# CrystalSixone/VLN-MAGIC

Measured on AMD Instinct MI355X. Metric: trajectory-steps/sec (whole node), MAGIC-S R2R pretrain, higher is better.
Workload: dtype bf16

## Files before the change

### vln-magic_amd/csrc/encoder.hip

```cpp
#include "enc_common.hpp"
#include <cstdlib>
#include <cstring>

template <typename Hh> struct EncLayerT {
  const Hh* Wqkv; const float* bqkv;
  const Hh* Wo; const float* bo; const float* g1; const float* be1;
  const Hh* W1; const float* bi;
  const Hh* W2; const float* bo2; const float* g2; const float* be2;
  Hh *qkv, *P, *Pd, *ctx, *a, *z, *g, *out;
  float *rstd_a, *rstd_o;
  unsigned site_attn, site_ao, site_out, pad_;
};
template <typename Hh> struct EncSegT { const Hh* x; const unsigned char* kmask; int nsamp, N, ldp, nlayers; EncLayerT<Hh> L[6]; };
template <typename Hh> struct EncParamsT {
  EncSegT<Hh> seg[2]; int nseg; float p_attn, p_hidden, eps, scale; const unsigned* seed;
  unsigned* sync; int sync_words, pad2_;
};
typedef EncParamsT<bf16> EncParams; typedef EncSegT<bf16> EncSeg; typedef EncLayerT<bf16> EncLayer;
#define F(f) ABI_VIEW(EncLayer, magic_enc_layer, f)
F(Wqkv) F(bqkv) F(Wo) F(bo) F(g1) F(be1) F(W1) F(bi) F(W2) F(bo2) F(g2) F(be2) F(qkv) F(P) F(Pd) F(ctx) F(a) F(z) F(g) F(out) F(rstd_a) F(rstd_o)
F(site_attn) F(site_ao) F(site_out) F(pad_)
#undef F
#define F(f) ABI_VIEW(EncSeg, magic_enc_seg, f)
F(x) F(kmask) F(nsamp) F(N) F(ldp) F(nlayers) F(L)
// ... 1139 lines not shown
    {
      f32x4 acc[NRT][3];
#pragma unroll
      for (int i = 0; i < NRT; ++i)
#pragma unroll
        for (int ct = 0; ct < 3; ++ct) acc[i][ct] = (f32x4){0.f, 0.f, 0.f, 0.f};
#pragma unroll
      for (int ks = 0; ks < 4; ++ks) {
#pragma unroll
        for (int i = 0; i < NRT; ++i) {
          const h16x8<Hh> a = lfrag(sX, XS, i * 16, ks * 32, lane);
#pragma unroll
          for (int ct = 0; ct < 3; ++ct) acc[i][ct] = emma(a, bw[ct][ks], acc[i][ct]);
        }
        KSTEP_FENCE();
      }
#pragma unroll
      for (int ct = 0; ct < 3; ++ct) {
        const int col = (3 * w + ct) * 16 + c16;
#pragma unroll
        for (int i = 0; i < NRT; ++i)
#pragma unroll
          for (int r = 0; r < 4; ++r) sQKV[(i * 16 + 4 * g + r) * QS + col] = from_f<Hh>(acc[i][ct][r] + pb_qkv[ct]);
      }
    }
    h16x8<Hh> wo[4], wq[4];
#pragma unroll
    for (int ks = 0; ks < 4; ++ks) { wo[ks] = gfrag(L.Wo, EH, w * 16, ks * 32, lane); wq[ks] = gfrag(L.Wq, EH, w * 16, ks * 32, lane); }
    __syncthreads();
    copy_out(sQKV, QS, L.qkv + qbase * 3 * EH, 3 * EH, Nq, 3 * EH, tid);
    dd.site = L.site_attn; dd.p = p.p_attn;
    const DropState dsa = drop_init(dd);
    Hh* sPw = sP + w * 16 * PSW;
    for (int u = w; u < ENH * NRT; u += NWAVE)
      attn_unit<NRT>(sQKV, sPw, sA, L.P, L.Pd, u / NRT, u % NRT, Nq, Nq, sg.ldps, qbias, sg.dist, sw, sb, samp, p.scale, dsa, lane);
    __syncthreads();
    copy_out(sA, XS, L.ctx + qbase * EH, EH, Nq, EH, tid);
    {
      f32x4 acc[NRT];
      proj16<NRT>(acc, sA, wo, lane);
      dd.site = L.site_ao; dd.p = p.p_hidden;
      const DropState dsh = drop_init(dd);
      add_norm<NRT, MAXROWS>(acc, pb_o, pg_1, pe_1, sX, red, sA, L.rstd_a, Nq, qbase, p.eps, dsh, w, lane);
    }
    h16x8<Hh> wkv[2][4];
#pragma unroll
    for (int ct = 0; ct < 2; ++ct)
#pragma unroll
      for (int ks = 0; ks < 4; ++ks) wkv[ct][ks] = gfrag(L.Wkv, EH, (2 * w + ct) * 16, ks * 32, lane);
    __syncthreads();
    copy_out(sA, XS, L.a + qbase * EH, EH, Nq, EH, tid);
    {
      f32x4 acc[NRT];
      proj16<NRT>(acc, sA, wq, lane);
#pragma unroll
      for (int i = 0; i < NRT; ++i)
#pragma unroll
        for (int r = 0; r < 4; ++r) sQKV[(i * 16 + 4 * g + r) * QS + colw] = from_f<Hh>(acc[i][r] + pb_q);
    }
    {
      f32x4 acc[NKT][2];
#pragma unroll
      for (int i = 0; i < NKT; ++i)
#pragma unroll
        for (int ct = 0; ct < 2; ++ct) acc[i][ct] = (f32x4){0.f, 0.f, 0.f, 0.f};
      const Hh* cx = sg.cx + kbase * EH;
#pragma unroll
      for (int ks = 0; ks < 4; ++ks) {
#pragma unroll
        for (int i = 0; i < NKT; ++i) {
          const int row = min(i * 16 + c16, Nk - 1);
          const h16x8<Hh> a = *(const h16x8<Hh>*)(cx + (long long)row * EH + ks * 32 + 8 * g);
#pragma unroll
          for (int ct = 0; ct < 2; ++ct) acc[i][ct] = emma(a, wkv[ct][ks], acc[i][ct]);
        }
        KSTEP_FENCE();
      }
#pragma unroll
      for (int ct = 0; ct < 2; ++ct) {
        const int col = EH + (2 * w + ct) * 16 + c16;
#pragma unroll
        for (int i = 0; i < NKT; ++i)
#pragma unroll
          for (int r = 0; r < 4; ++r) {
            const int row = i * 16 + 4 * g + r;
            sQKV[row * QS + col] = (row < Nk) ? from_f<Hh>(acc[i][ct][r] + pb_kv[ct]) : (Hh)0.0f;
          }
      }
    }
    for (int id = tid; id < (KROWS - NKT * 16) * (256 / 8); id += NWAVE * 64) {
      const int r = NKT * 16 + id / 32, c = EH + (id % 32) * 8;
      h16x8<Hh> zv;
#pragma unroll
      for (int e = 0; e < 8; ++e) zv[e] = (Hh)0.0f;
      *(h16x8<Hh>*)(sQKV + r * QS + c) = zv;
    }
    h16x8<Hh> woc[4];
#pragma unroll
    for (int ks = 0; ks < 4; ++ks) woc[ks] = gfrag(L.Woc, EH, w * 16, ks * 32, lane);
    h16x8<Hh> w1[4][4];
#pragma unroll
    for (int ct = 0; ct < 4; ++ct)
#pragma unroll
      for (int ks = 0; ks < 4; ++ks) w1[ct][ks] = gfrag(L.W1, EH, (4 * w + ct) * 16, ks * 32, lane);
    __syncthreads();
    copy_out(sQKV, QS, L.q + qbase * EH, EH, Nq, EH, tid);
    copy_out(sQKV + EH, QS, L.kv + kbase * 2 * EH, 2 * EH, Nk, 2 * EH, tid);
    dd.site = L.site_cattn; dd.p = p.p_attn;
    const DropState dsc = drop_init(dd);
    for (int u = w; u < ENH * NRT; u += NWAVE)
      attn_unit<NKT>(sQKV, sPw, sX, L.Pc, L.Pdc, u / NRT, u % NRT, Nq, Nk, sg.ldpc, cbias, nullptr, 0.f, 0.f, samp, p.scale, dsc, lane);
    __syncthreads();
    copy_out(sX, XS, L.cctx + qbase * EH, EH, Nq, EH, tid);
    {
      f32x4 acc[NRT];
      proj16<NRT>(acc, sX, woc, lane);
      dd.site = L.site_co; dd.p = p.p_hidden;
      const DropState dsh = drop_init(dd);
      add_norm<NRT, MAXROWS>(acc, pb_oc, pg_c, pe_c, sA, red, sX, L.rstd_c, Nq, qbase, p.eps, dsh, w, lane);
    }
    __syncthreads();
    copy_out(sX, XS, L.c + qbase * EH, EH, Nq, EH, tid);
    h16x8<Hh> w2[16];
    {
      f32x4 acc[NRT][4];
#pragma unroll
      for (int i = 0; i < NRT; ++i)
#pragma unroll
        for (int ct = 0; ct < 4; ++ct) acc[i][ct] = (f32x4){0.f, 0.f, 0.f, 0.f};
#pragma unroll
      for (int ks = 0; ks < 4; ++ks) {
#pragma unroll
        for (int i = 0; i < NRT; ++i) {
          const h16x8<Hh> a = lfrag(sX, XS, i * 16, ks * 32, lane);
#pragma unroll
          for (int ct = 0; ct < 4; ++ct) acc[i][ct] = emma(a, w1[ct][ks], acc[i][ct]);
        }
        KSTEP_FENCE();
      }
#pragma unroll
      for (int ks = 0; ks < 16; ++ks) w2[ks] = gfrag(L.W2, EI, w * 16, ks * 32, lane);
#pragma unroll
      for (int ct = 0; ct < 4; ++ct) {
        const int col = (4 * w + ct) * 16 + c16;
#pragma unroll
        for (int i = 0; i < NRT; ++i)
#pragma unroll
          for (int r = 0; r < 4; ++r) {
            acc[i][ct][r] += pb_ffn[ct];
            sG[(i * 16 + 4 * g + r) * GS + col] = from_f<Hh>(acc[i][ct][r]);
          }
      }
      __syncthreads();
      copy_out(sG, GS, L.z + qbase * EI, EI, Nq, EI, tid);
#pragma unroll
      for (int ct = 0; ct < 4; ++ct)
#pragma unroll
        for (int i = 0; i < NRT; ++i)
#pragma unroll
          for (int r = 0; r < 4; ++r) acc[i][ct][r] = gelu_fast(acc[i][ct][r]);
      __syncthreads();
#pragma unroll
      for (int ct = 0; ct < 4; ++ct) {
        const int col = (4 * w + ct) * 16 + c16;
#pragma unroll
        for (int i = 0; i < NRT; ++i)
#pragma unroll
          for (int r = 0; r < 4; ++r) sG[(i * 16 + 4 * g + r) * GS + col] = from_f<Hh>(acc[i][ct][r]);
      }
    }
    __syncthreads();
    copy_out(sG, GS, L.g + qbase * EI, EI, Nq, EI, tid);
    {
      f32x4 acc[NRT];
#pragma unroll
      for (int i = 0; i < NRT; ++i) acc[i] = (f32x4){0.f, 0.f, 0.f, 0.f};
#pragma unroll
      for (int ks = 0; ks < 16; ++ks) {
#pragma unroll
        for (int i = 0; i < NRT; ++i) acc[i] = emma(lfrag(sG, GS, i * 16, ks * 32, lane), w2[ks], acc[i]);
        if ((ks & 1) == 1) KSTEP_FENCE();
      }
      dd.site = L.site_out; dd.p = p.p_hidden;
      const DropState dsh = drop_init(dd);
      add_norm<NRT, MAXROWS>(acc, pb_2, pg_2, pe_2, sX, red, sX, L.rstd_o, Nq, qbase, p.eps, dsh, w, lane);
    }
    __syncthreads();
    copy_out(sX, XS, L.out + qbase * EH, EH, Nq, EH, tid);
  }
}

template <int NKT, typename Hh>
__device__ __forceinline__ void rs_attn(Hh* sQ, const Hh* sK, const Hh* sV, float* sS, Hh* sPd, const float (&kbias)[NKT], const int Nk, const int kmax,
                                        const float* dist, const float sw, const float sb, const int q0, const int nq, const int Nq,
                                        Hh* Pg, Hh* Pdg, const int ldp, const long long samp, const float scale, const DropState& dsa,
                                        const int tid, const int w, const int lane) {
  const int g = lane >> 4, c16 = lane & 15;
  const int NKP = (Nk + 31) / 32 * 32;
  for (int u = w; u < ENH * NKT; u += NWAVE) {
    const int h = u / NKT, j = u % NKT;
    f32x4 sc = (f32x4){0.f, 0.f, 0.f, 0.f};
#pragma unroll
    for (int ks = 0; ks < 2; ++ks) sc = emma(lfrag(sQ, XS, 0, h * EHD + ks * 32, lane), lfrag(sK, XS, j * 16, h * EHD + ks * 32, lane), sc);
    const int key = j * 16 + c16;
    float mb = 0.f;
#pragma unroll
    for (int jj = 0; jj < NKT; ++jj) mb = (jj == j) ? kbias[jj] : mb;
#pragma unroll
    for (int r = 0; r < 4; ++r) {
      float x = sc[r] * scale + mb;
      if (dist && key < Nk) { const int qrow = min(q0 + 4 * g + r, Nq - 1); x += sw * dist[((long long)samp * Nq + qrow) * Nk + key] + sb; }
      sS[(h * 16 + 4 * g + r) * RS_SS + key] = key < Nk ? x : -3.0e38f;
    }
  }
  __syncthreads();
  {
    const int rr = 4 * w + g, h = rr >> 4, ql = rr & 15;
    float e[NKT], mx = -3.0e38f;
#pragma unroll
    for (int j = 0; j < NKT; ++j) { e[j] = sS[rr * RS_SS + j * 16 + c16]; mx = fmaxf(mx, e[j]); }
    mx = g16_max(mx);
    float sum = 0.f;
#pragma unroll
    for (int j = 0; j < NKT; ++j) { e[j] = (j * 16 + c16) < Nk ? __expf(e[j] - mx) : 0.f; sum += e[j]; }
    sum = 1.0f / g16_sum(sum);
    Hh* pc = (Hh*)(sS + rr * RS_SS);
    Hh* pd = sPd + rr * RS_PP;
#pragma unroll
    for (int j = 0; j < NKT; ++j) {
      const int key = j * 16 + c16;
      const float pv = e[j] * sum;
      pc[key] = from_f<Hh>(pv);
      if (dsa.on) {
        const unsigned idx = (unsigned)(((((long long)samp * ENH + h) * Nq + q0 + ql) * Nk) + key);
        pd[key] = from_f<Hh>((ql < nq && key < Nk) ? pv * drop_mul(dsa, idx) : 0.f);
      }
    }
    if (NKT * 16 < NKP && c16 < NKP - NKT * 16) { pc[NKT * 16 + c16] = (Hh)0.0f; if (dsa.on) pd[NKT * 16 + c16] = (Hh)0.0f; }
  }
  __syncthreads();
  {
    const int cpr = ldp / 8;
    for (int id = tid; id < ENH * nq * cpr; id += NWAVE * 64) {
      const int h = id / (nq * cpr), rem = id % (nq * cpr), r = rem / cpr, c = (rem % cpr) * 8;
      const long long go = (((long long)samp * ENH + h) * Nq + q0 + r) * ldp + c;
      *(h16x8<Hh>*)(Pg + go) = *(const h16x8<Hh>*)((const Hh*)(sS + (h * 16 + r) * RS_SS) + c);
      if (dsa.on && Pdg) *(h16x8<Hh>*)(Pdg + go) = *(const h16x8<Hh>*)(sPd + (h * 16 + r) * RS_PP + c);
    }
  }
  {
    const int h = w >> 2, jd = w & 3;
    const Hh* pa = dsa.on ? sPd + h * 16 * RS_PP : (const Hh*)(sS + h * 16 * RS_SS);
    const int pp = dsa.on ? RS_PP : 2 * RS_SS;
    f32x4 o = (f32x4){0.f, 0.f, 0.f, 0.f};
    for (int ks = 0; ks < NKP / 32; ++ks)
      o = emma(lfrag(pa, pp, 0, ks * 32, lane), tfrag_clamp(sV + h * EHD, XS, jd * 16, ks * 32, lane, kmax), o);
#pragma unroll
    for (int r = 0; r < 4; ++r) sQ[(4 * g + r) * XS + h * EHD + jd * 16 + c16] = from_f<Hh>(o[r]);
  }
  __syncthreads();
}

template <int NRT, typename Hh>
__device__ __forceinline__ void xenc_rs_body(const XParamsT<Hh>& p, const XSegT<Hh>& sg, const int samp, const int tile, const int ntile,
                                             unsigned* cnt, unsigned* err, unsigned char* smem) {
  constexpr int NKT = 5;
  Hh* sK = (Hh*)smem;
  Hh* sV = sK + 80 * XS;
  Hh* sU = sV + 81 * XS;
  Hh* sX = sU;
  float* sS = (float*)sU;
  Hh* sPd = sU + 2 * 16 * RS_SS * 2;
  Hh* sG = sU;
  Hh* sZ = sK;
  Hh* sQ = sU + 80 * XS;
  Hh* sO = sQ + 16 * XS;
  Hh* sA = sO + 16 * XS;
  float* red = (float*)(sA + 16 * XS);
  const int tid = threadIdx.x, lane0 = tid & 63, w = __builtin_amdgcn_readfirstlane(tid >> 6);
  const int Nq = sg.Nq, Nk = sg.Nk;
  const long long qbase = (long long)samp * Nq, kbase = (long long)samp * Nk;
  const int r0 = tile * 16, nq = min(16, Nq - r0);
  const long long row0 = qbase + r0;
  if (tid < XS / 8) {
    h16x8<Hh> zv;
#pragma unroll
    for (int e = 0; e < 8; ++e) zv[e] = (Hh)0.0f;
    *(h16x8<Hh>*)(sV + RS_ZROW * XS + tid * 8) = zv;
  }
  DropDesc dd;
  dd.seed = p.seed;
  float qbias[NRT], cbias[NKT];
#pragma unroll
  for (int j = 0; j < NRT; ++j) {
    const int key = j * 16 + (lane0 & 15);
    qbias[j] = (key < Nq && sg.qmask && !sg.qmask[qbase + key]) ? -10000.0f : 0.f;
  }
#pragma unroll
  for (int j = 0; j < NKT; ++j) {
    const int key = j * 16 + (lane0 & 15);
    cbias[j] = (key < Nk && sg.cmask && !sg.cmask[kbase + key]) ? -10000.0f : 0.f;
  }
  const float sw = sg.dist ? sg.sprel_w[0] : 0.f, sb = sg.dist ? sg.sprel_b[0] : 0.f;
  for (int l = 0; l < sg.nlayers; ++l) {
    const XLayerT<Hh>& L = sg.L[l];
    int lane = lane0;
    asm volatile("" : "+v"(lane));
    const int g = lane >> 4, c16 = lane & 15;
    const int colw = w * 16 + c16;
    const float pb_q0 = L.bqkv[colw], pb_kv0 = L.bqkv[EH + (2 * w) * 16 + c16], pb_kv1 = L.bqkv[EH + (2 * w + 1) * 16 + c16];
    const float pb_ck0 = L.bkv[(2 * w) * 16 + c16], pb_ck1 = L.bkv[(2 * w + 1) * 16 + c16];
    float pb_ffn[4];
#pragma unroll
    for (int ct = 0; ct < 4; ++ct) pb_ffn[ct] = L.bi[(4 * w + ct) * 16 + c16];
    const float pb_o = L.bo[colw], pg_1 = L.g1[colw], pe_1 = L.be1[colw], pb_q = L.bq[colw];
    const float pb_oc = L.boc[colw], pg_c = L.gc[colw], pe_c = L.bec[colw];
    const float pb_2 = L.bo2[colw], pg_2 = L.g2[colw], pe_2 = L.be2[colw];
    h16x8<Hh> wq[4], wkv[2][4];
#pragma unroll
    for (int ks = 0; ks < 4; ++ks) {
      wq[ks] = gfrag(L.Wqkv, EH, w * 16, ks * 32, lane);
      wkv[0][ks] = gfrag(L.Wqkv, EH, EH + (2 * w) * 16, ks * 32, lane);
      wkv[1][ks] = gfrag(L.Wqkv, EH, EH + (2 * w + 1) * 16, ks * 32, lane);
    }
    if (l > 0) {
      if (tid == 0) {
        gu32_t* c = (gu32_t*)(cnt + (long long)samp * 6 + (l - 1));
        unsigned spins = 0;
        while (__hip_atomic_load(c, __ATOMIC_RELAXED, __HIP_MEMORY_SCOPE_AGENT) < (unsigned)ntile) {
          __builtin_amdgcn_s_sleep(4);
          if (++spins > RS_SPIN_MAX) { enc_give_up((gu32_t*)err); break; }
        }
      }
      __syncthreads();
    }
    {
      const Hh* x = (l == 0 ? sg.x : sg.L[l - 1].out) + qbase * EH;
      const auto rsrc = __builtin_amdgcn_make_buffer_rsrc((void*)x, 0, Nq * EH * 2, 0x00020000);
      for (int id = tid; id < NRT * 16 * (EH / 8); id += NWAVE * 64) {
        const int r = id / (EH / 8), c = (id % (EH / 8)) * 8;
        const u32x4 v = __builtin_amdgcn_raw_buffer_load_b128(rsrc, (r * EH + c) * 2, 0, 16);
        *(u32x4*)(sX + r * XS + c) = v;
        if (r >= r0 && r < r0 + 16) *(u32x4*)(sO + (r - r0) * XS + c) = v;
      }
    }
    __syncthreads();
    {
      f32x4 acc[NRT][2], aq = (f32x4){0.f, 0.f, 0.f, 0.f};
#pragma unroll
      for (int i = 0; i < NRT; ++i) { acc[i][0] = (f32x4){0.f, 0.f, 0.f, 0.f}; acc[i][1] = (f32x4){0.f, 0.f, 0.f, 0.f}; }
#pragma unroll
      for (int ks = 0; ks < 4; ++ks) {
#pragma unroll
        for (int i = 0; i < NRT; ++i) {
          const h16x8<Hh> a = lfrag(sX, XS, i * 16, ks * 32, lane);
          acc[i][0] = emma(a, wkv[0][ks], acc[i][0]);
          acc[i][1] = emma(a, wkv[1][ks], acc[i][1]);
        }
        aq = emma(lfrag(sO, XS, 0, ks * 32, lane), wq[ks], aq);
        KSTEP_FENCE();
      }
      Hh* dst = (w < 4 ? sK : sV) + ((2 * w) & 7) * 16 + c16;
#pragma unroll
      for (int i = 0; i < NRT; ++i)
#pragma unroll
        for (int r = 0; r < 4; ++r) {
          dst[(i * 16 + 4 * g + r) * XS] = from_f<Hh>(acc[i][0][r] + pb_kv0);
          dst[(i * 16 + 4 * g + r) * XS + 16] = from_f<Hh>(acc[i][1][r] + pb_kv1);
        }
#pragma unroll
      for (int r = 0; r < 4; ++r) sQ[(4 * g + r) * XS + colw] = from_f<Hh>(aq[r] + pb_q0);
    }
    h16x8<Hh> wo[4], wcq[4];
#pragma unroll
    for (int ks = 0; ks < 4; ++ks) { wo[ks] = gfrag(L.Wo, EH, w * 16, ks * 32, lane); wcq[ks] = gfrag(L.Wq, EH, w * 16, ks * 32, lane); }
    __syncthreads();
    {
      Hh* qg = L.qkv + row0 * 3 * EH;
      for (int id = tid; id < nq * 48; id += NWAVE * 64) {
        const int r = id / 48, c = (id % 48) * 8;
        const Hh* src = c < EH ? sQ + r * XS + c : (c < 2 * EH ? sK + (r0 + r) * XS + (c - EH) : sV + (r0 + r) * XS + (c - 2 * EH));
        *(h16x8<Hh>*)(qg + (long long)r * 3 * EH + c) = *(const h16x8<Hh>*)src;
      }
    }
    dd.site = L.site_attn; dd.p = p.p_attn;
    const DropState dsa = drop_init(dd);
    rs_attn<NRT>(sQ, sK, sV, sS, sPd, qbias, Nq, NRT * 16, sg.dist, sw, sb, r0, nq, Nq, L.P, L.Pd, sg.ldps, samp, p.scale, dsa, tid, w, lane);
    copy_tile<false>(sQ, XS, L.ctx + row0 * EH, EH, nq, EH, tid);
    {
      f32x4 acc = (f32x4){0.f, 0.f, 0.f, 0.f};
#pragma unroll
      for (int ks = 0; ks < 4; ++ks) acc = emma(lfrag(sQ, XS, 0, ks * 32, lane), wo[ks], acc);
      dd.site = L.site_ao; dd.p = p.p_hidden;
      const DropState dsh = drop_init(dd);
      add_norm16(acc, pb_o, pg_1, pe_1, sO, red, sA, L.rstd_a, nq, row0, p.eps, dsh, w, lane);
    }
    h16x8<Hh> wck[2][4];
#pragma unroll
    for (int ct = 0; ct < 2; ++ct)
#pragma unroll
      for (int ks = 0; ks < 4; ++ks) wck[ct][ks] = gfrag(L.Wkv, EH, (2 * w + ct) * 16, ks * 32, lane);
    __syncthreads();
    copy_tile<false>(sA, XS, L.a + row0 * EH, EH, nq, EH, tid);
    {
      f32x4 aq = (f32x4){0.f, 0.f, 0.f, 0.f};
#pragma unroll
      for (int ks = 0; ks < 4; ++ks) aq = emma(lfrag(sA, XS, 0, ks * 32, lane), wcq[ks], aq);
#pragma unroll
      for (int r = 0; r < 4; ++r) sQ[(4 * g + r) * XS + colw] = from_f<Hh>(aq[r] + pb_q);
      f32x4 acc[NKT][2];
#pragma unroll
      for (int i = 0; i < NKT; ++i) { acc[i][0] = (f32x4){0.f, 0.f, 0.f, 0.f}; acc[i][1] = (f32x4){0.f, 0.f, 0.f, 0.f}; }
      const Hh* cx = sg.cx + kbase * EH;
#pragma unroll
      for (int ks = 0; ks < 4; ++ks) {
#pragma unroll
        for (int i = 0; i < NKT; ++i) {
          const int row = min(i * 16 + c16, Nk - 1);
          const h16x8<Hh> a = *(const h16x8<Hh>*)(cx + (long long)row * EH + ks * 32 + 8 * g);
          acc[i][0] = emma(a, wck[0][ks], acc[i][0]);
          acc[i][1] = emma(a, wck[1][ks], acc[i][1]);
        }
        KSTEP_FENCE();
      }
      Hh* dst = (w < 4 ? sK : sV) + ((2 * w) & 7) * 16 + c16;
#pragma unroll
      for (int i = 0; i < NKT; ++i)
#pragma unroll
        for (int r = 0; r < 4; ++r) {
          const int row = i * 16 + 4 * g + r;
          dst[row * XS] = row < Nk ? from_f<Hh>(acc[i][0][r] + pb_ck0) : (Hh)0.0f;
          dst[row * XS + 16] = row < Nk ? from_f<Hh>(acc[i][1][r] + pb_ck1) : (Hh)0.0f;
        }
    }
    h16x8<Hh> woc[4], w1[4][4];
#pragma unroll
    for (int ks = 0; ks < 4; ++ks) woc[ks] = gfrag(L.Woc, EH, w * 16, ks * 32, lane);
#pragma unroll
    for (int ct = 0; ct < 4; ++ct)
#pragma unroll
      for (int ks = 0; ks < 4; ++ks) w1[ct][ks] = gfrag(L.W1, EH, (4 * w + ct) * 16, ks * 32, lane);
    __syncthreads();
    copy_tile<false>(sQ, XS, L.q + row0 * EH, EH, nq, EH, tid);
    for (int kt = tile; kt * 16 < Nk; kt += ntile) {
      const int nr = min(16, Nk - kt * 16);
      Hh* kg = L.kv + (kbase + kt * 16) * 2 * EH;
      for (int id = tid; id < nr * 32; id += NWAVE * 64) {
        const int r = id / 32, c = (id % 32) * 8;
        const Hh* src = c < EH ? sK + (kt * 16 + r) * XS + c : sV + (kt * 16 + r) * XS + (c - EH);
        *(h16x8<Hh>*)(kg + (long long)r * 2 * EH + c) = *(const h16x8<Hh>*)src;
      }
    }
    dd.site = L.site_cattn; dd.p = p.p_attn;
    const DropState dsc = drop_init(dd);
    rs_attn<NKT>(sQ, sK, sV, sS, sPd, cbias, Nk, NKT * 16, nullptr, 0.f, 0.f, r0, nq, Nq, L.Pc, L.Pdc, sg.ldpc, samp, p.scale, dsc, tid, w, lane);
    copy_tile<false>(sQ, XS, L.cctx + row0 * EH, EH, nq, EH, tid);
    {
      f32x4 acc = (f32x4){0.f, 0.f, 0.f, 0.f};
#pragma unroll
      for (int ks = 0; ks < 4; ++ks) acc = emma(lfrag(sQ, XS, 0, ks * 32, lane), woc[ks], acc);
      dd.site = L.site_co; dd.p = p.p_hidden;
      const DropState dsh = drop_init(dd);
      add_norm16(acc, pb_oc, pg_c, pe_c, sA, red, sO, L.rstd_c, nq, row0, p.eps, dsh, w, lane);
    }
    __syncthreads();
    copy_tile<false>(sO, XS, L.c + row0 * EH, EH, nq, EH, tid);
    h16x8<Hh> w2[16];
    {
      f32x4 acc[4];
#pragma unroll
      for (int ct = 0; ct < 4; ++ct) acc[ct] = (f32x4){0.f, 0.f, 0.f, 0.f};
#pragma unroll
      for (int ks = 0; ks < 4; ++ks) {
        const h16x8<Hh> a = lfrag(sO, XS, 0, ks * 32, lane);
#pragma unroll
        for (int ct = 0; ct < 4; ++ct) acc[ct] = emma(a, w1[ct][ks], acc[ct]);
      }
#pragma unroll
      for (int ks = 0; ks < 16; ++ks) w2[ks] = gfrag(L.W2, EI, w * 16, ks * 32, lane);
#pragma unroll
      for (int ct = 0; ct < 4; ++ct) {
        const int col = (4 * w + ct) * 16 + c16;
#pragma unroll
        for (int r = 0; r < 4; ++r) {
          const float zv = acc[ct][r] + pb_ffn[ct];
          sZ[(4 * g + r) * GS + col] = from_f<Hh>(zv);
          sG[(4 * g + r) * GS + col] = from_f<Hh>(gelu_fast(zv));
        }
      }
    }
    __syncthreads();
    copy_tile<false>(sZ, GS, L.z + row0 * EI, EI, nq, EI, tid);
    copy_tile<false>(sG, GS, L.g + row0 * EI, EI, nq, EI, tid);
    {
      f32x4 acc = (f32x4){0.f, 0.f, 0.f, 0.f};
#pragma unroll
      for (int ks = 0; ks < 16; ++ks) acc = emma(lfrag(sG, GS, 0, ks * 32, lane), w2[ks], acc);
      dd.site = L.site_out; dd.p = p.p_hidden;
      const DropState dsh = drop_init(dd);
      add_norm16(acc, pb_2, pg_2, pe_2, sO, red, sA, L.rstd_o, nq, row0, p.eps, dsh, w, lane);
    }
    __syncthreads();
    copy_tile<true>(sA, XS, L.out + row0 * EH, EH, nq, EH, tid);
    asm volatile("s_waitcnt vmcnt(0)" ::: "memory");
    __syncthreads();
    if (tid == 0 && l + 1 < sg.nlayers) __hip_atomic_fetch_add((gu32_t*)(cnt + (long long)samp * 6 + l), 1u, __ATOMIC_RELAXED, __HIP_MEMORY_SCOPE_AGENT);
  }
}

template <typename Hh>
__global__ __launch_bounds__(512) void xencoder_rs_kernel(XParamsT<Hh> p, int nt0, int nt1) {
  extern __shared__ __attribute__((aligned(16))) unsigned char enc_smem[];
  int b = blockIdx.x, s = 0, nt = nt0;
  unsigned* cnt = p.sync + 4;
  if (b >= p.seg[0].nsamp * nt0) { b -= p.seg[0].nsamp * nt0; s = 1; nt = nt1; cnt += 6ll * p.seg[0].nsamp; }
  const XSegT<Hh>& sg = p.seg[s];
  const int samp = b / nt, tile = b - samp * nt;
  if (nt <= 3) xenc_rs_body<3>(p, sg, samp, tile, nt, cnt, p.sync, enc_smem);
  else xenc_rs_body<5>(p, sg, samp, tile, nt, cnt, p.sync, enc_smem);
}

template <typename Hh>
__global__ __launch_bounds__(512) void xencoder_fwd_kernel(XParamsT<Hh> p) {
  extern __shared__ __attribute__((aligned(16))) unsigned char enc_smem[];
  int b = blockIdx.x, s = 0;
  if (b >= p.seg[0].nsamp) { b -= p.seg[0].nsamp; s = 1; }
  const XSegT<Hh>& sg = p.seg[s];
  const int nrt = max(2, (sg.Nq + 15) / 16);
  switch (nrt) {
    case 2: xenc_body<2>(p, sg, b, enc_smem); break;
    case 3: xenc_body<3>(p, sg, b, enc_smem); break;
    case 4: xenc_body<4>(p, sg, b, enc_smem); break;
    default: xenc_body<5>(p, sg, b, enc_smem); break;
  }
}

extern "C" int magic_xencoder_supported(int dtype, int H, int I, int nh, int Nq, int Nk, int nlayers) {
  return dtype_is16(dtype) && H == EH && I == EI && nh == ENH && Nq >= 1 && Nq <= MAXROWS && Nk >= 1 && Nk <= MAXROWS && nlayers >= 1 && nlayers <= 3;
}
extern "C" int magic_xencoder_params_bytes() { return (int)sizeof(XParams); }

extern "C" int magic_xencoder_fwd(int dtype, const void* params, int nbytes, void* stream) {
  if (!params || nbytes != (int)sizeof(XParams) || !dtype_is16(dtype)) return MAGIC_ERR_ARG;
  XParams p;
  memcpy(&p, params, sizeof(p));
  if (p.nseg < 1 || p.nseg > 2) return MAGIC_ERR_ARG;
  if (!drop_args_ok(p.seed, p.p_attn) || !drop_args_ok(p.seed, p.p_hidden)) return MAGIC_ERR_ARG;
  int blocks = 0;
  for (int s = 0; s < 2; ++s) {
    XSeg& sg = p.seg[s];
    if (s >= p.nseg) { sg.nsamp = 0; continue; }
    if (sg.nsamp <= 0 || sg.Nq < 1 || sg.Nq > MAXROWS || sg.Nk < 1 || sg.Nk > MAXROWS || sg.nlayers < 1 || sg.nlayers > 3 || !sg.x || !sg.cx) return MAGIC_ERR_ARG;
    if (sg.ldps < sg.Nq || (sg.ldps & 7) || sg.ldps > KROWS || sg.ldpc < sg.Nk || (sg.ldpc & 7) || sg.ldpc > KROWS) return MAGIC_ERR_ARG;
    if ((long long)sg.nsamp * ENH * sg.Nq * MAXROWS > 0xFFFFFFFFll) return MAGIC_ERR_ARG;
    if (((uintptr_t)sg.x & 15) || ((uintptr_t)sg.cx & 15)) return MAGIC_ERR_ARG;
    if (sg.dist && (!sg.sprel_w || !sg.sprel_b)) return MAGIC_ERR_ARG;
    for (int l = 0; l < sg.nlayers; ++l) {
      const XLayer& L = sg.L[l];
      const void* req[] = {L.Wqkv, L.bqkv, L.Wo, L.bo, L.g1, L.be1, L.Wq, L.bq, L.Wkv, L.bkv, L.Woc, L.boc, L.gc, L.bec, L.W1, L.bi, L.W2, L.bo2, L.g2, L.be2,
                           L.qkv, L.P, L.ctx, L.a, L.rstd_a, L.q, L.kv, L.Pc, L.cctx, L.c, L.rstd_c, L.z, L.g, L.out, L.rstd_o};
      for (const void* q : req)
        if (!q) return MAGIC_ERR_ARG;
      const void* al[] = {L.Wqkv, L.Wo, L.Wq, L.Wkv, L.Woc, L.W1, L.W2, L.qkv, L.P, L.Pd, L.ctx, L.a, L.q, L.kv, L.Pc, L.Pdc, L.cctx, L.c, L.z, L.g, L.out};
      for (const void* q : al)
        if ((uintptr_t)q & 15) return MAGIC_ERR_ARG;
      if (p.p_attn > 0.f && (!L.Pd || !L.Pdc)) return MAGIC_ERR_ARG;
    }
    blocks += sg.nsamp;
  }
  if (p.sync) {
    const int nt0 = (p.seg[0].Nq + 15) / 16, nt1 = p.nseg > 1 ? (p.seg[1].Nq + 15) / 16 : 1;
    const int ns1 = p.nseg > 1 ? p.seg[1].nsamp : 0;
    const long long words = 4 + 6ll * (p.seg[0].nsamp + ns1);
    if (p.sync_words < words || ((uintptr_t)p.sync & 15)) return MAGIC_ERR_ARG;
    static int ncu = 0;
    if (!ncu) { hipDeviceProp_t pr; int d = 0; (void)hipGetDevice(&d); ncu = (hipGetDeviceProperties(&pr, d) == hipSuccess) ? pr.multiProcessorCount : 256; }
    const int grid = p.seg[0].nsamp * nt0 + ns1 * nt1;
    if (grid <= ncu && grid > blocks) {
      static bool rs_attr = false;
      if (!rs_attr) {
        (void)hipFuncSetAttribute((const void*)xencoder_rs_kernel<bf16>, hipFuncAttributeMaxDynamicSharedMemorySize, (int)enc_rs_lds_bytes());
        (void)hipFuncSetAttribute((const void*)xencoder_rs_kernel<f16>, hipFuncAttributeMaxDynamicSharedMemorySize, (int)enc_rs_lds_bytes());
        rs_attr = true;
      }
      if (hipMemsetAsync(p.sync, 0, (size_t)((words + 3) / 4 * 4) * sizeof(unsigned), (hipStream_t)stream) != hipSuccess) return MAGIC_ERR_LAUNCH;
      if (dtype == DT_BF16) hipLaunchKernelGGL(xencoder_rs_kernel<bf16>, dim3(grid), dim3(512), enc_rs_lds_bytes(), (hipStream_t)stream, p, nt0, nt1);
      else { XParamsT<f16> pf; static_assert(sizeof(pf) == sizeof(p), "layout"); memcpy(&pf, &p, sizeof(pf)); hipLaunchKernelGGL(xencoder_rs_kernel<f16>, dim3(grid), dim3(512), enc_rs_lds_bytes(), (hipStream_t)stream, pf, nt0, nt1); }
      return launch_status();
    }
    if (hipMemsetAsync(p.sync, 0, 16, (hipStream_t)stream) != hipSuccess) return MAGIC_ERR_LAUNCH;
  }
  const size_t shm = enc_lds_bytes();
  static bool attr_set = false;
  if (!attr_set) {
    (void)hipFuncSetAttribute((const void*)xencoder_fwd_kernel<bf16>, hipFuncAttributeMaxDynamicSharedMemorySize, (int)shm);
    (void)hipFuncSetAttribute((const void*)xencoder_fwd_kernel<f16>, hipFuncAttributeMaxDynamicSharedMemorySize, (int)shm);
    attr_set = true;
  }
  if (dtype == DT_BF16) hipLaunchKernelGGL(xencoder_fwd_kernel<bf16>, dim3(blocks), dim3(512), shm, (hipStream_t)stream, p);
  else { XParamsT<f16> pf; static_assert(sizeof(pf) == sizeof(p), "layout"); memcpy(&pf, &p, sizeof(pf)); hipLaunchKernelGGL(xencoder_fwd_kernel<f16>, dim3(blocks), dim3(512), shm, (hipStream_t)stream, pf); }
  return launch_status();
}
```

Before: 189,000.

## Precompute cross-attention K/V for later layers once, split across tiles

Every block used to recompute the full cross-attention K/V projection of the fixed context for every layer. Now, before the layer loop, each tile projects only its assigned key tiles for layers 1 and up and stores them to global `L.kv`, using a per-layer rotation to spread the work. Inside the loop, layers after the first just load the precomputed K/V from global with buffer loads into shared memory. This removes repeated MFMA work and context reads, but makes blocks depend on K/V written by other blocks, so correctness relies on some cross-block ordering that the code shown does not make explicit.

```diff
diff --git a/vln-magic_amd/csrc/encoder.hip b/vln-magic_amd/csrc/encoder.hip
--- a/vln-magic_amd/csrc/encoder.hip
+++ b/vln-magic_amd/csrc/encoder.hip
@@ -1465,6 +1465,55 @@
     cbias[j] = (key < Nk && sg.cmask && !sg.cmask[kbase + key]) ? -10000.0f : 0.f;
   }
   const float sw = sg.dist ? sg.sprel_w[0] : 0.f, sb = sg.dist ? sg.sprel_b[0] : 0.f;
+  const int nkt = (Nk + 15) / 16;
+  for (int lu = 1; lu < sg.nlayers; ++lu) {
+    const int k0 = ((tile - lu) % ntile + ntile) % ntile;
+    if (k0 >= nkt) continue;
+    const XLayerT<Hh>& L = sg.L[lu];
+    const int g = lane0 >> 4, c16 = lane0 & 15;
+    h16x8<Hh> wck[2][4], a[NKT][4];
+#pragma unroll
+    for (int ct = 0; ct < 2; ++ct)
+#pragma unroll
+      for (int ks = 0; ks < 4; ++ks) wck[ct][ks] = gfrag(L.Wkv, EH, (2 * w + ct) * 16, ks * 32, lane0);
+    const float pb_ck0 = L.bkv[(2 * w) * 16 + c16], pb_ck1 = L.bkv[(2 * w + 1) * 16 + c16];
+    const Hh* cx = sg.cx + kbase * EH;
+#pragma unroll
+    for (int j = 0; j < NKT; ++j) {
+      const int kt = k0 + j * ntile;
+      if (kt < nkt) {
+        const int row = min(kt * 16 + c16, Nk - 1);
+#pragma unroll
+        for (int ks = 0; ks < 4; ++ks) a[j][ks] = *(const h16x8<Hh>*)(cx + (long long)row * EH + ks * 32 + 8 * g);
+      }
+    }
+#pragma unroll
+    for (int j = 0; j < NKT; ++j) {
+      const int kt = k0 + j * ntile;
+      if (kt < nkt) {
+        f32x4 c0 = (f32x4){0.f, 0.f, 0.f, 0.f}, c1 = (f32x4){0.f, 0.f, 0.f, 0.f};
+#pragma unroll
+        for (int ks = 0; ks < 4; ++ks) { c0 = emma(a[j][ks], wck[0][ks], c0); c1 = emma(a[j][ks], wck[1][ks], c1); }
+        Hh* dst = (w < 4 ? sK : sV) + kt * 16 * XS + ((2 * w) & 7) * 16 + c16;
+#pragma unroll
+        for (int r = 0; r < 4; ++r) {
+          dst[(4 * g + r) * XS] = from_f<Hh>(c0[r] + pb_ck0);
+          dst[(4 * g + r) * XS + 16] = from_f<Hh>(c1[r] + pb_ck1);
+        }
+      }
+    }
+    __syncthreads();
+    for (int kt = k0; kt < nkt; kt += ntile) {
+      const int nr = min(16, Nk - kt * 16);
+      const auto rsrc = __builtin_amdgcn_make_buffer_rsrc((void*)(L.kv + (kbase + kt * 16) * 2 * EH), 0, nr * 2 * EH * 2, 0x00020000);
+      for (int id = tid; id < nr * 32; id += NWAVE * 64) {
+        const int r = id / 32, c = (id % 32) * 8;
+        const Hh* src = c < EH ? sK + (kt * 16 + r) * XS + c : sV + (kt * 16 + r) * XS + (c - EH);
+        __builtin_amdgcn_raw_buffer_store_b128(*(const u32x4*)src, rsrc, (r * 2 * EH + c) * 2, 0, 16);
+      }
+    }
+    __syncthreads();
+  }
   for (int l = 0; l < sg.nlayers; ++l) {
     const XLayerT<Hh>& L = sg.L[l];
     int lane = lane0;
@@ -1558,11 +1607,6 @@
       const DropState dsh = drop_init(dd);
       add_norm16(acc, pb_o, pg_1, pe_1, sO, red, sA, L.rstd_a, nq, row0, p.eps, dsh, w, lane);
     }
-    h16x8<Hh> wck[2][4];
-#pragma unroll
-    for (int ct = 0; ct < 2; ++ct)
-#pragma unroll
-      for (int ks = 0; ks < 4; ++ks) wck[ct][ks] = gfrag(L.Wkv, EH, (2 * w + ct) * 16, ks * 32, lane);
     __syncthreads();
     copy_tile<false>(sA, XS, L.a + row0 * EH, EH, nq, EH, tid);
     {
@@ -1571,30 +1615,47 @@
       for (int ks = 0; ks < 4; ++ks) aq = emma(lfrag(sA, XS, 0, ks * 32, lane), wcq[ks], aq);
 #pragma unroll
       for (int r = 0; r < 4; ++r) sQ[(4 * g + r) * XS + colw] = from_f<Hh>(aq[r] + pb_q);
-      f32x4 acc[NKT][2];
-#pragma unroll
-      for (int i = 0; i < NKT; ++i) { acc[i][0] = (f32x4){0.f, 0.f, 0.f, 0.f}; acc[i][1] = (f32x4){0.f, 0.f, 0.f, 0.f}; }
-      const Hh* cx = sg.cx + kbase * EH;
-#pragma unroll
-      for (int ks = 0; ks < 4; ++ks) {
+      if (l > 0) {
+        const auto rsrc = __builtin_amdgcn_make_buffer_rsrc((void*)(L.kv + kbase * 2 * EH), 0, Nk * 2 * EH * 2, 0x00020000);
+        u32x4 kvr[NKT];
+#pragma unroll
+        for (int i = 0; i < NKT; ++i) kvr[i] = __builtin_amdgcn_raw_buffer_load_b128(rsrc, (tid + i * NWAVE * 64) * 16, 0, 16);
 #pragma unroll
         for (int i = 0; i < NKT; ++i) {
-          const int row = min(i * 16 + c16, Nk - 1);
-          const h16x8<Hh> a = *(const h16x8<Hh>*)(cx + (long long)row * EH + ks * 32 + 8 * g);
-          acc[i][0] = emma(a, wck[0][ks], acc[i][0]);
-          acc[i][1] = emma(a, wck[1][ks], acc[i][1]);
-        }
-        KSTEP_FENCE();
-      }
-      Hh* dst = (w < 4 ? sK : sV) + ((2 * w) & 7) * 16 + c16;
-#pragma unroll
-      for (int i = 0; i < NKT; ++i)
-#pragma unroll
-        for (int r = 0; r < 4; ++r) {
-          const int row = i * 16 + 4 * g + r;
-          dst[row * XS] = row < Nk ? from_f<Hh>(acc[i][0][r] + pb_ck0) : (Hh)0.0f;
-          dst[row * XS + 16] = row < Nk ? from_f<Hh>(acc[i][1][r] + pb_ck1) : (Hh)0.0f;
-        }
+          const int id = tid + i * NWAVE * 64, r = id / 32, c = (id % 32) * 8;
+          *(u32x4*)(c < EH ? sK + r * XS + c : sV + r * XS + (c - EH)) = kvr[i];
+        }
+      } else {
+        h16x8<Hh> wck[2][4];
+#pragma unroll
+        for (int ct = 0; ct < 2; ++ct)
+#pragma unroll
+          for (int ks = 0; ks < 4; ++ks) wck[ct][ks] = gfrag(L.Wkv, EH, (2 * w + ct) * 16, ks * 32, lane);
+        f32x4 acc[NKT][2];
+#pragma unroll
+        for (int i = 0; i < NKT; ++i) { acc[i][0] = (f32x4){0.f, 0.f, 0.f, 0.f}; acc[i][1] = (f32x4){0.f, 0.f, 0.f, 0.f}; }
+        const Hh* cx = sg.cx + kbase * EH;
+#pragma unroll
+        for (int ks = 0; ks < 4; ++ks) {
+#pragma unroll
+          for (int i = 0; i < NKT; ++i) {
+            const int row = min(i * 16 + c16, Nk - 1);
+            const h16x8<Hh> a = *(const h16x8<Hh>*)(cx + (long long)row * EH + ks * 32 + 8 * g);
+            acc[i][0] = emma(a, wck[0][ks], acc[i][0]);
+            acc[i][1] = emma(a, wck[1][ks], acc[i][1]);
+          }
+          KSTEP_FENCE();
+        }
+        Hh* dst = (w < 4 ? sK : sV) + ((2 * w) & 7) * 16 + c16;
+#pragma unroll
+        for (int i = 0; i < NKT; ++i)
+#pragma unroll
+          for (int r = 0; r < 4; ++r) {
+            const int row = i * 16 + 4 * g + r;
+            dst[row * XS] = row < Nk ? from_f<Hh>(acc[i][0][r] + pb_ck0) : (Hh)0.0f;
+            dst[row * XS + 16] = row < Nk ? from_f<Hh>(acc[i][1][r] + pb_ck1) : (Hh)0.0f;
+          }
+      }
     }
     h16x8<Hh> woc[4], w1[4][4];
 #pragma unroll
@@ -1605,15 +1666,16 @@
       for (int ks = 0; ks < 4; ++ks) w1[ct][ks] = gfrag(L.W1, EH, (4 * w + ct) * 16, ks * 32, lane);
     __syncthreads();
     copy_tile<false>(sQ, XS, L.q + row0 * EH, EH, nq, EH, tid);
-    for (int kt = tile; kt * 16 < Nk; kt += ntile) {
-      const int nr = min(16, Nk - kt * 16);
-      Hh* kg = L.kv + (kbase + kt * 16) * 2 * EH;
-      for (int id = tid; id < nr * 32; id += NWAVE * 64) {
-        const int r = id / 32, c = (id % 32) * 8;
-        const Hh* src = c < EH ? sK + (kt * 16 + r) * XS + c : sV + (kt * 16 + r) * XS + (c - EH);
-        *(h16x8<Hh>*)(kg + (long long)r * 2 * EH + c) = *(const h16x8<Hh>*)src;
-      }
-    }
+    if (l == 0)
+      for (int kt = tile; kt * 16 < Nk; kt += ntile) {
+        const int nr = min(16, Nk - kt * 16);
+        Hh* kg = L.kv + (kbase + kt * 16) * 2 * EH;
+        for (int id = tid; id < nr * 32; id += NWAVE * 64) {
+          const int r = id / 32, c = (id % 32) * 8;
+          const Hh* src = c < EH ? sK + (kt * 16 + r) * XS + c : sV + (kt * 16 + r) * XS + (c - EH);
+          *(h16x8<Hh>*)(kg + (long long)r * 2 * EH + c) = *(const h16x8<Hh>*)src;
+        }
+      }
     dd.site = L.site_cattn; dd.p = p.p_attn;
     const DropState dsc = drop_init(dd);
     rs_attn<NKT>(sQ, sK, sV, sS, sPd, cbias, Nk, NKT * 16, nullptr, 0.f, 0.f, r0, nq, Nq, L.Pc, L.Pdc, sg.ldpc, samp, p.scale, dsc, tid, w, lane);
```

After: 189,700, median of 6. About the same (+0.4%).
